# mikeferguson/ndt_2d

Hardware: AMD Instinct MI355X
Metric: pose-candidates x beams scored per second (higher is better)
Workload: dtype f64

## Files before the change

### experiments/asm_loop_mix.py

```python
#!/usr/bin/env python3
import collections
import hashlib
import json
import os
import re
import subprocess
import sys
import tempfile

R = os.path.dirname(os.path.dirname(os.path.abspath(__file__)))
KERNELS = [
    ("ndt2d_match_lane.hip", "match_lane_compact_kernel", r"25match_lane_compact_kernelILb1ELb1EEE"),
    ("ndt2d_match_lane.hip", "match_lane_compact_parts_kernel", r"31match_lane_compact_parts_kernelILb1EEE"),
    ("ndt2d_match_small.hip", "match_small_kernel", r"18match_small_kernelILb1ELb1ELb1EEE"),
    ("ndt2d_poses_compact.hip", "score_poses_compact_kernel", r"26score_poses_compact_kernelILi256ELb1ELb1ELb0EEE"),
]


def kernel_lines(path, pattern):
    out, on = [], False
    for line in open(path):
        if not on:
            if re.match(r"^_Z\w*%s\w*:" % pattern, line):
                on = True
            continue
        out.append(line)
        if line.strip().startswith("s_endpgm"):
            break
# ... 139 lines not shown
```

### experiments/lane_path_mix.py

```python
#!/usr/bin/env python3
import json
import os
import sys

R = os.path.dirname(os.path.dirname(os.path.abspath(__file__)))
paths_file = sys.argv[1] if len(sys.argv) > 1 else os.path.join(R, "profiles", "r06_lane_paths.json")
pmc_file = sys.argv[2] if len(sys.argv) > 2 else os.path.join(R, "profiles", "r06_pmc.json")
issue = json.load(open(os.path.join(R, "profiles", "r05_ubench_issue.json")))
CYC = issue["cycles"]
CLS = {k: ([c for c in v.get("counted_by", []) if not c.startswith("(")] or ["other"])[0]
       for k, v in issue["instructions"].items()}

P = {
    "lookup_group (per 8 beams)": [("v_add_f64", 8), ("v_perm_b32", 8), ("v_max_u32", 1), ("v_max3_u32", 3),
                                    ("v_cmp_le_u32 vcc", 1)],
    "live_group (8 live tests)": [("v_cmp_le_u32 vcc", 8)],
    "live_beam": [("v_and_b32", 1), ("v_cmp_le_u32 vcc", 1)],
    "near_test": [("v_cmp_gt_u16 vcc", 2), ("v_perm_b32", 1)],
    "exact_evaluation": [("v_add_f64", 2),
                         ("v_lshrrev_b32_sdwa", 2), ("v_mul_u32_u24", 1), ("v_add3_u32", 1), ("v_cndmask_b32 sgpr", 1),
                         ("v_lshl_add_u32", 1), ("v_mad_u32_u24", 1),
                         ("v_add_f64", 5), ("v_mul_f64", 6), ("v_cmp_lt_f64 vcc", 1)],
    "reference_index (extra)": [("v_add_f64", 2), ("v_mul_f64", 2), ("v_cmp_lt_f64 vcc", 4), ("v_cvt_u32_f64", 2),
                                ("v_mad_u64_u32", 1), ("v_mov_b32 from sgpr", 1), ("v_cndmask_b32 vcc", 1),
                                ("v_lshrrev_b32_sdwa", -2), ("v_mul_u32_u24", -1), ("v_add3_u32", -1),
                                ("v_cndmask_b32 sgpr", -1)],
    "exp_and_add": [("v_max_f64", 1), ("v_mul_f64", 1), ("v_rndne_f64", 1), ("v_fmac_f64", 2), ("v_fma_f64", 11),
                    ("v_cvt_i32_f64", 1), ("v_cmp_lt_f64 vcc", 1), ("v_ldexp_f64", 1), ("v_add_f64", 1)],
    "skip_refresh": [("v_frexp_exp_i32_f64", 1), ("v_add_u32", 2), ("v_mov_b32", 2), ("v_cvt_f64_i32", 1),
                     ("v_fma_f64", 1), ("v_cmp_lt_f64 vcc", 2), ("v_cndmask_b32 vcc", 2), ("v_ceil_f64", 1),
                     ("v_cvt_i32_f64", 1), ("v_max_u32", 1), ("v_min_u32", 1), ("v_lshlrev_b32", 1)],
}

doc = json.load(open(paths_file))
n = doc["counts"]
execs = {
    "lookup_group (per 8 beams)": n["beams_in_lookup_groups"] / 8.0,
    "live_group (8 live tests)": n["groups_with_a_live_lane"],
    "live_beam": n["beams_with_a_live_lane"],
    "near_test": n["live_beams_near_possible"],
    "exact_evaluation": n["exact_evaluations"],
# ... 57 lines not shown
```

### ndt_2d_amd/build.py

```python
import os
import subprocess
import sys

_PKG = os.path.dirname(os.path.abspath(__file__))
_ROOT = os.path.dirname(_PKG)
_CSRC = os.path.join(_PKG, "csrc")
LIB_PATH = os.path.join(_PKG, "libndt2d_hip.so")

BUILD_INFO_SOURCE = "ndt2d_build_info.cpp"
SOURCES = ["ndt2d_kernels.hip", "ndt2d_match_lane.hip", "ndt2d_match_small.hip", "ndt2d_poses_compact.hip", "ndt2d_build.hip", "ndt2d_motion.hip", "ndt2d_scan.hip", "ndt2d_occupancy.hip", "ndt2d_exchange.hip",
           "device/ndt2d_context.hip", "device/ndt2d_context_grid.hip", "device/ndt2d_context_search.hip", "device/ndt2d_context_poses.hip", "device/ndt2d_context_scan.hip",
           "resample/ndt2d_resample.hip", "occupancy_map/ndt2d_occupancy_map.hip", "seed/ndt2d_seed.hip", "clearance/ndt2d_clearance.hip", "cluster/ndt2d_cluster.hip", "build_small/ndt2d_build_small.hip", "closure/ndt2d_closure.hip", "starts/ndt2d_starts.hip", "wide/ndt2d_wide.hip", "scans/ndt2d_scans.hip", "refine/ndt2d_refine.hip", "verify/ndt2d_verify.hip", "posegraph/ndt2d_posegraph.hip", "posegraph/ndt2d_posegraph_robust.hip", "posegraph/ndt2d_posegraph_marginals.hip", "covariance/ndt2d_covariance.hip", "direct/ndt2d_direct.hip", "sparse/ndt2d_sparse.hip", "sparsecov/ndt2d_sparsecov.hip", "ndt2d_host.cpp",
           "host/ndt2d_host_ndt.cpp", "host/ndt2d_multi.cpp", "host/ndt2d_batched.cpp", "host/ndt2d_kld.cpp", "host/ndt2d_synth.cpp"]
HEADERS = [os.path.join(_CSRC, "ndt2d_kernels.h"), os.path.join(_CSRC, "ndt2d_device_fn.h"), os.path.join(_CSRC, "ndt2d_lane_fn.h"), os.path.join(_CSRC, "ndt2d_near_bits.h"), os.path.join(_CSRC, "ndt2d_pretest_level.h"), os.path.join(_CSRC, "ndt2d_poses_fn.h"), os.path.join(_CSRC, "ndt2d_exchange.h"), os.path.join(_CSRC, "ndt2d_eigen2.h"), os.path.join(_CSRC, "build_small", "ndt2d_build_fn.h"), os.path.join(_CSRC, "build_small", "ndt2d_build_small_fn.h"), os.path.join(_CSRC, "ndt2d_workers.h"), os.path.join(_CSRC, "ndt2d_guard.h"), os.path.join(_CSRC, "batch", "ndt2d_sum_chunks.h"), os.path.join(_CSRC, "batch", "ndt2d_walk_fn.h"), os.path.join(_CSRC, "batch", "ndt2d_job_groups.h"), os.path.join(_CSRC, "batch", "ndt2d_stage_layout.h"), os.path.join(_CSRC, "batch", "ndt2d_batch_search.h"), os.path.join(_CSRC, "batch", "ndt2d_installed_map.h"), os.path.join(_CSRC, "batch", "ndt2d_batch_state.h"), os.path.join(_CSRC, "batch", "ndt2d_batch_host.h"), os.path.join(_CSRC, "batch", "ndt2d_refine_jobs.h"), os.path.join(_CSRC, "refine", "ndt2d_refine_step.h"), os.path.join(_CSRC, "verify", "ndt2d_verify_ray.h"), os.path.join(_CSRC, "posegraph", "ndt2d_posegraph_fn.h"), os.path.join(_CSRC, "posegraph", "ndt2d_posegraph_chain.h"), os.path.join(_CSRC, "posegraph", "ndt2d_posegraph_loss.h"), os.path.join(_CSRC, "posegraph", "ndt2d_posegraph_relative.h"), os.path.join(_CSRC, "posegraph", "ndt2d_posegraph_kernel.h"), os.path.join(_CSRC, "posegraph", "ndt2d_posegraph_state.h"), os.path.join(_CSRC, "posegraph", "ndt2d_posegraph_args.h"), os.path.join(_CSRC, "covariance", "ndt2d_covariance_plan.h"), os.path.join(_CSRC, "covariance", "ndt2d_covariance_kernel.h"), os.path.join(_CSRC, "covariance", "ndt2d_covariance_launch.h"), os.path.join(_CSRC, "direct", "ndt2d_direct_step.h"), os.path.join(_CSRC, "direct", "ndt2d_direct_plan.h"), os.path.join(_CSRC, "direct", "ndt2d_direct_kernel.h"), os.path.join(_CSRC, "sparse", "ndt2d_sparse_plan.h"), os.path.join(_CSRC, "sparse", "ndt2d_sparse_schur.h"), os.path.join(_CSRC, "sparse", "ndt2d_sparse_kernel.h"), os.path.join(_CSRC, "sparsecov", "ndt2d_sparsecov_plan.h"), os.path.join(_CSRC, "sparsecov", "ndt2d_sparsecov_select.h"), os.path.join(_CSRC, "sparsecov", "ndt2d_sparsecov_kernel.h"), os.path.join(_CSRC, "seed", "ndt2d_seed_fn.h"), os.path.join(_CSRC, "clearance", "ndt2d_clearance_fn.h"), os.path.join(_CSRC, "cluster", "ndt2d_cluster_fn.h"), os.path.join(_CSRC, "wide", "ndt2d_wide_fn.h"), os.path.join(_CSRC, "closure", "ndt2d_closure_jobs.h"), os.path.join(_CSRC, "host", "ndt2d_host_ndt.h"), os.path.join(_CSRC, "host", "ndt2d_matcher_state.h"), os.path.join(_CSRC, "host", "ndt2d_job_batch.h"), os.path.join(_CSRC, "device", "ndt2d_context.h"), os.path.join(_CSRC, "refine", "ndt2d_refine_kernel.h"), os.path.join(_CSRC, "verify", "ndt2d_verify_kernel.h"), os.path.join(_CSRC, "particles", "ndt2d_philox.h"), os.path.join(_CSRC, "particles", "ndt2d_compact_fn.h"), os.path.join(_CSRC, "particles", "ndt2d_compact.h"), os.path.join(_CSRC, "particles", "ndt2d_key_table.h"), os.path.join(_CSRC, "particles", "ndt2d_device_object.h"), os.path.join(_ROOT, "include", "ndt2d_hip.h")]
ARCH = "gfx950"
FLAGS = ["-O3", "-std=c++17", "-ffp-contract=off", "-fPIC", "-Wall", "-Wextra",
         "-Wno-unused-parameter"]


SHA_MARKER = b"NDT2D_SOURCE_SHA256="


def source_sha256():
    import hashlib
    h = hashlib.sha256()
    paths = [os.path.join(_CSRC, s) for s in SOURCES + [BUILD_INFO_SOURCE]] + HEADERS
    for path in sorted(paths, key=os.path.basename):
        h.update(os.path.basename(path).encode() + b"\0")
        with open(path, "rb") as f:
# ... 178 lines not shown
```

### ndt_2d_amd/csrc/ndt2d_lane_fn.h

```cpp
#ifndef NDT2D_LANE_FN_H_
#define NDT2D_LANE_FN_H_

#include <cmath>

#include "ndt2d_device_fn.h"
#include "ndt2d_near_bits.h"
#include "ndt2d_pretest_level.h"

namespace ndt2d
{

namespace
{

constexpr int kPatch = 8;
#ifndef NDT2D_LANE_UNROLL
#define NDT2D_LANE_UNROLL 8
#endif
constexpr int kUnroll = NDT2D_LANE_UNROLL;
#ifndef NDT2D_LANE_NEAR_BITS
#define NDT2D_LANE_NEAR_BITS 1
#endif
constexpr double kFracScale = 65536.0;
constexpr int kMapStride = 256;
constexpr int kMaxMapCells = 256;
constexpr double kBoxMargin = 1.0 / 1024.0;
constexpr double kTwo24 = 16777216.0;
constexpr double kTwo52 = 4503599627370496.0;
constexpr double kNearBias = kNearUnits * (kTwo24 + 1.0);
static_assert(kNearUnits == 4 && kNearPatch == kPatch, "near_boundary() tests the biased fraction against 2 * kNearUnits");

struct LaneGeom
{
  int32_t pad;
// ... 272 lines not shown
  do {                                                                                        \
    if (g_lane_hist != nullptr && (threadIdx.x & 63u) == 0) atomicAdd(g_lane_hist + (slot), static_cast<double>(amount)); \
  } while (0)
#else
#define NDT2D_PATH(slot, amount) do {} while (0)
#endif

struct LaneCtx
{
  uint32_t rank_address;
  uint32_t lds_cells_address;
  uint32_t sub_log2;
  uint32_t exact_index;
  uint32_t idx_bias;
  uint32_t size_x;
};

__device__ __forceinline__ uint32_t lds_byte_at(uint32_t address)
{
  typedef const __attribute__((address_space(3))) uint8_t * lds_byte_ptr;
  return *reinterpret_cast<lds_byte_ptr>(address);
}

__device__ __forceinline__ uint32_t lds_u16_at(uint32_t address)
{
  typedef const __attribute__((address_space(3))) uint16_t * lds_u16_ptr;
  return *reinterpret_cast<lds_u16_ptr>(address);
}

__device__ __forceinline__ uint64_t near_boundary(uint32_t v)
{
  uint64_t lanes;
  asm("v_cmp_gt_u16_e64 %0, 8, %1" : "=s"(lanes) : "v"(v));
  return lanes;
}

__device__ __forceinline__ uint2 lds_two_dwords_at(uint32_t address)
{
  typedef const __attribute__((address_space(3), aligned(4))) uint32_t * lds_u32_ptr;
  const lds_u32_ptr p = reinterpret_cast<lds_u32_ptr>(address);
  return make_uint2(p[0], p[1]);
}
// ... 59 lines not shown
  v = min(v, __builtin_amdgcn_update_dpp(v, v, kDppRowMirror, 0xf, 0xf, false));
  v = min(v, __builtin_amdgcn_update_dpp(v, v, kDppRowBcast15, 0xa, 0xf, false));
  v = min(v, __builtin_amdgcn_update_dpp(v, v, kDppRowBcast31, 0xc, 0xf, false));
  return static_cast<uint32_t>(__builtin_amdgcn_readlane(v, kWave - 1));
}

__device__ __forceinline__ double lds_record_exponent(uint32_t cells_address, uint32_t idx,
                                                      double px, double py)
{
  typedef const __attribute__((address_space(3), aligned(16))) double * lds_double_ptr;
  const lds_double_ptr rec = reinterpret_cast<lds_double_ptr>(
    __umul24(idx, static_cast<uint32_t>(kCellDoubles * sizeof(double))) + cells_address);
  return record_exponent(rec[0], rec[1], rec[2], rec[3], rec[4], px, py);
}

struct SkipState
{
  double skip_below;
  uint32_t skip_level;
};

__device__ __forceinline__ SkipState skip_state(double sum, int32_t no_skip)
{
  SkipState s;
  if (no_skip)
  {
    s.skip_below = -HUGE_VAL;
    s.skip_level = 0;
    return s;
  }
  s.skip_below = negligible_below(sum);
  const int32_t l = static_cast<int32_t>(ceil(s.skip_below)) + 63;
  s.skip_level = static_cast<uint32_t>(min(max(l, 1), 63)) << 2;
  return s;
}

template <int U, bool POW2, bool LDS_RECORDS, bool SCALAR_ROWS = true, bool COMPACT = false>
__device__ __forceinline__ bool lane_beams(const GridDesc & g, const LaneCtx & c,
                                           const double4 (&o)[U], double dx, double dy,
                                           double dxy, double & sum, SkipState & skip,
                                           int32_t no_skip, uint32_t near_possible = ~0u)
{
  const double skip_below = skip.skip_below;
  const uint32_t skip_level = skip.skip_level;
  uint32_t lo[U], hi[U], m[U];
  uint32_t top = 0;
#pragma unroll
  for (int u = 0; u < U; ++u)
  {
    const double s = o[u].z + dxy;
    lo[u] = static_cast<uint32_t>(__double2loint(s));
    hi[u] = static_cast<uint32_t>(__double2hiint(s));
// ... 27 lines not shown
            (near_boundary(lo[u]) | near_boundary(fy) | ((no_skip | c.exact_index) != 0 ? ~0ull : 0ull)) & live_mask;
        }
        const uint64_t occ_lanes = __builtin_amdgcn_ballot_w64(occ);
        const uint64_t occ_mask = occ_lanes & live_mask;
#ifdef NDT2D_LANE_NO_EXACT
        if ((occ_mask | near_mask) == 0x1234567ull)
#else
        if ((occ_mask | near_mask) != 0ull)
#endif
        {
          NDT2D_PATH(205, 1);
          if (near_mask != 0ull) NDT2D_PATH(206, 1);
          const double px = o[u].x + dx;
          const double py = o[u].y + dy;
          uint32_t idx;
          if (near_mask != 0ull)
          {
            idx = cell_index<POW2>(g, px, py);
          }
          else
          {
            const uint32_t col = ((lo[u] >> 16) & 0xffu) >> c.sub_log2;
            const uint32_t row = ((hi[u] >> 8) & 0xffu) >> c.sub_log2;
            const uint32_t cell = __umul24(row, c.size_x) + (col - c.idx_bias);
            if (COMPACT)
            {
              asm("v_cndmask_b32 %0, -1, %1, %2" : "=v"(idx) : "v"(cell), "s"(occ_lanes));
            }
            else
            {
              idx = occ ? cell : g.ncell;
            }
          }
          if (COMPACT) idx = lds_u16_at(c.rank_address + 2u * idx);
          const double e = LDS_RECORDS ? lds_record_exponent(c.lds_cells_address, idx, px, py)
                                       : indexed_exponent<false>(g, nullptr, idx, px, py);
#ifdef NDT2D_LANE_HIST
          if (g_lane_hist != nullptr)
          {
            const uint64_t flagged = occ_mask | near_mask;
            const uint64_t needed = __builtin_amdgcn_ballot_w64(!(e < skip_below)) & flagged;
            if ((threadIdx.x & 63u) == 0)
            {
              atomicAdd(g_lane_hist + __popcll(flagged), 1.0);
              atomicAdd(g_lane_hist + 70 + __popcll(needed), 1.0);
              atomicAdd(g_lane_hist + (needed != 0ull ? 140 : 141), 1.0);
            }
          }
#endif
          if (wave_any(!(e < skip_below)))
          {
// ... 124 lines not shown
```

### ndt_2d_amd/csrc/ndt2d_match_lane.hip

```cpp
#include <cmath>
#include <cstdlib>

#include <type_traits>

#include "ndt2d_lane_fn.h"

namespace ndt2d
{

namespace
{

constexpr uint32_t kDynamicItemsFromBeams = 256;
constexpr int kLaneThreads = 1024;
constexpr int kLaneThreadsSmall = 256;
#ifndef NDT2D_LANE_THREADS_COMPACT
#define NDT2D_LANE_THREADS_COMPACT 768
#endif
constexpr int kLaneThreadsCompact = NDT2D_LANE_THREADS_COMPACT;
#define NDT2D_LANE_COMPACT_WAVES_PER_EU (NDT2D_LANE_THREADS_COMPACT / 128)

#ifndef NDT2D_LANE_TABLE_2D
#define NDT2D_LANE_TABLE_2D 1
#endif
// ... 124 lines not shown

__device__ __forceinline__ double packed_offset(double dx, double dy, double inv_scaled)
{
  return rint(dy * inv_scaled) * kTwo24 + rint(dx * inv_scaled);
}

__device__ __forceinline__ double no_index_here()
{
  static_assert(kNoIndex == 1.0e308, "the literal below is 1.0e308");
  uint32_t lo, hi;
  asm volatile("v_mov_b32 %0, 0x85ebc8a0\n\tv_mov_b32 %1, 0x7fe1ccf3" : "=v"(lo), "=v"(hi));
  return __hiloint2double(static_cast<int>(hi), static_cast<int>(lo));
}

template <int THREADS, bool POW2, bool LDS_RECORDS, bool DYNAMIC_ITEMS, bool COMPACT, bool PARTS = false,
          bool STRIPS = false, bool NEAR = false>
__device__ __forceinline__ void match_lane_body(
  const MatchArgs & a, const double4 * __restrict__ outer, const uint8_t * __restrict__ map_image,
  const LaneGeom & geo)
{
  extern __shared__ __align__(16) double lds[];
  const GridDesc & g = a.grid;
#if defined(NDT2D_LANE_HIST) || defined(NDT2D_LANE_PATHS)
  if (blockIdx.x == 0 && threadIdx.x == 0) g_lane_hist = a.scores;
#endif
  uint8_t * lds_map = reinterpret_cast<uint8_t *>(lds);
  const uint32_t map_bytes = static_cast<uint32_t>(geo.map_h) * kMapStride;
  const uint32_t rank_bytes = COMPACT ? compact_rank_bytes(g.ncell) : 0u;
  double * lds_cells = lds + (map_bytes + rank_bytes) / sizeof(double);

  if (COMPACT)
  {
    const uint4 * src_rank = reinterpret_cast<const uint4 *>(g.cell_rank);
    uint4 * dst_rank = reinterpret_cast<uint4 *>(lds_map + map_bytes + kRankLead);
    for (uint32_t i = threadIdx.x; i < (rank_bytes - kRankLead) / 16; i += THREADS) dst_rank[i] = src_rank[i];
    if (threadIdx.x == 0)
    {
      reinterpret_cast<uint16_t *>(lds_map + map_bytes + kRankLead)[-1] = static_cast<uint16_t>(g.n_occ);
    }
    const uint32_t n2 = (g.n_occ + 1) * kCellDoubles / 2;
    const double2 * src = reinterpret_cast<const double2 *>(g.compact_records);
    double2 * dst = reinterpret_cast<double2 *>(lds_cells);
    for (uint32_t i = threadIdx.x; i < n2; i += THREADS) dst[i] = src[i];
  }
  else if (LDS_RECORDS)
  {
    stage_grid_to_lds(g, lds_cells);
  }
  {
    const uint32_t n16 = static_cast<uint32_t>(kMapStride) * geo.map_h / 16;
    const uint4 * src = reinterpret_cast<const uint4 *>(map_image);
    uint4 * dst = reinterpret_cast<uint4 *>(lds_map);
    for (uint32_t i = threadIdx.x; i < n16; i += THREADS) dst[i] = src[i];
// ... 1 lines not shown
  __syncthreads();

#ifdef NDT2D_LANE_TRACE
  const unsigned long long trace_t0 = wall_clock64();
  unsigned long long trace_last = trace_t0, trace_max = 0, trace_last_start = trace_t0;
  uint32_t trace_items = 0, trace_prev_item = 0, trace_flagged = 0;
#endif
  LaneCtx c;
  c.rank_address = map_bytes + (COMPACT ? kRankLead : 0u);
  c.lds_cells_address = map_bytes + rank_bytes;
  c.sub_log2 = static_cast<uint32_t>(geo.sub_log2);
  c.exact_index = geo.block_log2 > 0 ? 1u : 0u;
  c.idx_bias = static_cast<uint32_t>(geo.pad - geo.win_y0) * g.size_x +
               static_cast<uint32_t>(geo.pad - geo.win_x0);
  c.size_x = g.size_x;

  const uint32_t lane = threadIdx.x & (kWave - 1);
  const uint32_t wave = __builtin_amdgcn_readfirstlane(threadIdx.x >> 6);
  const uint32_t n_lin = a.n_lin;
  static_assert(!STRIPS || (DYNAMIC_ITEMS && !PARTS), "strip tiles: the unsplit dynamic-item forms only");
  const LaneTiling tiling = lane_tiling(n_lin, STRIPS);
  const uint32_t patches = tiling.per_theta;
  const uint32_t n_items = (a.th_end - a.th_begin) * patches * (PARTS ? a.beam_parts : 1u);
  constexpr uint32_t kLaneWaves = THREADS / kWave;
  const uint32_t n_workers = gridDim.x * kLaneWaves;
  const uint32_t worker = wave * gridDim.x + blockIdx.x;
  const uint64_t per_theta = static_cast<uint64_t>(n_lin) * n_lin;
  const uint32_t th_mid = (a.th_end - a.th_begin - 1u) / 2u;
  const uint32_t home_shard = blockIdx.x % kItemShards;
  const double inv_scaled = geo.inv_scaled;
// ... 104 lines not shown
          }
        }
      }
#ifdef NDT2D_LANE_TRACE
      trace_flagged += static_cast<uint32_t>(__popcll(can_score));
#endif
      const uint32_t chunk_end = min(b0 + static_cast<uint32_t>(kWave), beams_end);
      uint32_t b = b0;
      for (; b + kUnroll <= chunk_end; b += kUnroll, can_score >>= kUnroll, near_chunk >>= kUnroll)
      {
        if ((can_score & ((1ull << kUnroll) - 1ull)) == 0ull) continue;
        double4 o[kUnroll];
#pragma unroll
        for (int u = 0; u < kUnroll; ++u) o[u] = row[b + u];
        __builtin_amdgcn_s_setprio(3);
        if (lane_beams<kUnroll, POW2, LDS_RECORDS, true, COMPACT>(g, c, o, dx, dy, dxy, sum, skip, geo.no_skip,
                                                                  NEAR ? static_cast<uint32_t>(near_chunk) : ~0u))
        {
          level_min |= 1u;
        }
        __builtin_amdgcn_s_setprio(0);
      }
      for (; b < chunk_end; ++b, can_score >>= 1, near_chunk >>= 1)
      {
        if ((can_score & 1ull) == 0ull) continue;
        const double4 one[1] = {row[b]};
        if (lane_beams<1, POW2, LDS_RECORDS, true, COMPACT>(g, c, one, dx, dy, dxy, sum, skip, geo.no_skip,
                                                            NEAR ? static_cast<uint32_t>(near_chunk) : ~0u))
        {
          level_min |= 1u;
        }
      }
    }

    if (PARTS)
    {
      a.part_sums[static_cast<size_t>(item) * kWave + lane] = sum;
      uint32_t next = n_items;
      if (lane == kWave - 1)
      {
        for (uint32_t tried = 0; tried < kItemShards && next >= n_items; ++tried)
        {
          const uint32_t shard = (home_shard + tried) % kItemShards;
// ... 132 lines not shown
      out[1] = best_i;
#pragma unroll
      for (int k = 0; k < 10; ++k) out[2 + k] = acc[k];
    }
  }
}

template <int THREADS, bool POW2, bool LDS_RECORDS, bool DYNAMIC_ITEMS, bool STRIPS = false>
__global__ void __launch_bounds__(THREADS) match_lane_kernel(
  const MatchArgs a, const double4 * __restrict__ outer, const uint8_t * __restrict__ map_image,
  const LaneGeom geo)
{
  match_lane_body<THREADS, POW2, LDS_RECORDS, DYNAMIC_ITEMS, false, false, STRIPS>(a, outer, map_image, geo);
}

template <bool STRIPS, bool NEAR>
__global__ void __launch_bounds__(kLaneThreadsCompact) __attribute__((amdgpu_waves_per_eu(NDT2D_LANE_COMPACT_WAVES_PER_EU)))
match_lane_compact_kernel(const MatchArgs a, const double4 * __restrict__ outer,
                          const uint8_t * __restrict__ map_image, const LaneGeom geo)
{
  match_lane_body<kLaneThreadsCompact, true, true, true, true, false, STRIPS, NEAR>(a, outer, map_image, geo);
}

template <bool POW2, bool STRIPS, bool NEAR>
__global__ void __launch_bounds__(kLaneThreadsCompact) __attribute__((amdgpu_waves_per_eu(NDT2D_LANE_COMPACT_WAVES_PER_EU)))
match_lane_gather6_kernel(const MatchArgs a, const double4 * __restrict__ outer,
                          const uint8_t * __restrict__ map_image, const LaneGeom geo)
{
  match_lane_body<kLaneThreadsCompact, POW2, false, true, false, false, STRIPS, NEAR>(a, outer, map_image, geo);
}

template <bool NEAR>
__global__ void __launch_bounds__(kLaneThreadsCompact) __attribute__((amdgpu_waves_per_eu(NDT2D_LANE_COMPACT_WAVES_PER_EU)))
match_lane_compact_parts_kernel(const MatchArgs a, const double4 * __restrict__ outer,
                                const uint8_t * __restrict__ map_image, const LaneGeom geo)
{
  match_lane_body<kLaneThreadsCompact, true, true, true, true, true, false, NEAR>(a, outer, map_image, geo);
}

template <bool POW2, bool NEAR>
__global__ void __launch_bounds__(kLaneThreadsCompact) __attribute__((amdgpu_waves_per_eu(NDT2D_LANE_COMPACT_WAVES_PER_EU)))
match_lane_gather6_parts_kernel(const MatchArgs a, const double4 * __restrict__ outer,
                                const uint8_t * __restrict__ map_image, const LaneGeom geo)
{
  match_lane_body<kLaneThreadsCompact, POW2, false, true, false, true, false, NEAR>(a, outer, map_image, geo);
}

__global__ void __launch_bounds__(256) match_lane_combine_kernel(const MatchArgs a)
{
  const uint32_t lane = threadIdx.x & (kWave - 1);
  const uint32_t n_lin = a.n_lin;
  const uint32_t patches_1d = (n_lin + kPatch - 1) / kPatch;
// ... 183 lines not shown
  args.part_beams = part_beams;
  if (!(dynamic_items && beam_parts == 1)) geo.strips = 0;
  const bool strips = geo.strips != 0;
  const uint64_t n_tiles =
    static_cast<uint64_t>(args.th_end - args.th_begin) * lane_tiling(args.n_lin, geo.strips != 0).per_theta;
  const uint64_t n_sub_items = beam_parts > 1 ? n_items * beam_parts : n_tiles;

  const bool small = beam_parts == 1 && n_items <= static_cast<uint64_t>(cus) * (kLaneThreadsSmall / kWave);
  const uint32_t waves_per_block = (small ? kLaneThreadsSmall : kLaneThreads) / kWave;
  uint32_t blocks = static_cast<uint32_t>((n_tiles + waves_per_block - 1) / waves_per_block);
  uint32_t max_blocks = static_cast<uint32_t>(cus);
  if (max_blocks * waves_per_block > max_workers) max_blocks = max_workers / waves_per_block;
  if (blocks > max_blocks) blocks = max_blocks;
  if (blocks == 0) blocks = 1;
  const bool compact = !small && compact_possible;
  const bool gather6 = !compact && !small && gather6_possible;
  if (records_mode_out != nullptr)
  {
    *records_mode_out = (compact ? 2 : (lds_records ? 1 : 0)) | (geo.block_log2 > 0 ? 4 : 0);
  }
  if (compact || gather6)
  {
    lds_bytes = compact ? map_bytes + compact_bytes : map_bytes;
    const uint32_t wpb = kLaneThreadsCompact / kWave;
    blocks = static_cast<uint32_t>((n_sub_items + wpb - 1) / wpb);
    uint32_t cap = 2 * static_cast<uint32_t>(cus);
    if (cap * wpb > max_workers) cap = max_workers / wpb;
    if (blocks > cap) blocks = cap;
    if (blocks == 0) blocks = 1;
  }
#if NDT2D_LANE_TABLE_2D
  {
    const uint32_t beam_blocks = (args.n_beams + 255u) / 256u;
    const uint32_t map_blocks = static_cast<uint32_t>(map_bytes + 255) / 256u;
    uint32_t th_rows = args.th_end - args.th_begin;
    if (beam_blocks == 0 || th_rows == 0) return hipErrorInvalidValue;
    const uint32_t map_rows = (map_blocks + beam_blocks - 1u) / beam_blocks;
    if (map_rows >= kTableMaxRows) return hipErrorInvalidValue;
// ... 24 lines not shown
  auto pick = [&](auto threads_tag) -> hipError_t {
    constexpr int T = decltype(threads_tag)::value;
    auto with_items = [&](auto dyn_tag, auto strips_tag) -> hipError_t {
      constexpr bool D = decltype(dyn_tag)::value;
      constexpr bool S = decltype(strips_tag)::value;
      return lds_records ? (pow2 ? launch(match_lane_kernel<T, true, true, D, S>, T)
                                 : launch(match_lane_kernel<T, false, true, D, S>, T))
                         : (pow2 ? launch(match_lane_kernel<T, true, false, D, S>, T)
                                 : launch(match_lane_kernel<T, false, false, D, S>, T));
    };
    if (!dynamic_items) return with_items(std::false_type{}, std::false_type{});
    return strips ? with_items(std::true_type{}, std::true_type{}) : with_items(std::true_type{}, std::false_type{});
  };
  auto six_wave = [&](auto near_tag) -> hipError_t {
    constexpr bool N = decltype(near_tag)::value;
    if (beam_parts > 1)
    {
      return compact ? launch(match_lane_compact_parts_kernel<N>, kLaneThreadsCompact)
                     : (pow2 ? launch(match_lane_gather6_parts_kernel<true, N>, kLaneThreadsCompact)
                             : launch(match_lane_gather6_parts_kernel<false, N>, kLaneThreadsCompact));
    }
    if (compact)
    {
      return strips ? launch(match_lane_compact_kernel<true, N>, kLaneThreadsCompact)
                    : launch(match_lane_compact_kernel<false, N>, kLaneThreadsCompact);
    }
    return pow2 ? (strips ? launch(match_lane_gather6_kernel<true, true, N>, kLaneThreadsCompact)
                          : launch(match_lane_gather6_kernel<true, false, N>, kLaneThreadsCompact))
                : (strips ? launch(match_lane_gather6_kernel<false, true, N>, kLaneThreadsCompact)
                          : launch(match_lane_gather6_kernel<false, false, N>, kLaneThreadsCompact));
  };
  const bool near = lane_reads_near_bits(geo, args.n_lin);
  if (beam_parts > 1)
  {
    e = near ? six_wave(std::true_type{}) : six_wave(std::false_type{});
    if (e == hipSuccess)
    {
      hipLaunchKernelGGL(match_lane_combine_kernel, dim3(static_cast<uint32_t>((n_items + 3) / 4)), dim3(256),
                         0, stream, args);
      e = hipGetLastError();
// ... 22 lines not shown
```

Measured before the change: 3253 billion.

## Address compacted LDS records through a precomputed window address table

Builds an LDS table over the padded search window whose entries hold either the direct LDS byte address of each cell's compacted record (4-byte entries) or its rank (1-byte entries when there are at most 256 records). The lane loop can then take a cell's record address from one LDS load instead of computing a linear cell index, looking up a 16-bit rank and scaling it. The aim is to cut integer address arithmetic and one dependent LDS lookup from the hot beam loop. In exchange the block uses more LDS, which can lower occupancy, and pays a table build at kernel start; the table is chosen only when it fits and can be turned off by an environment knob.

```diff
diff --git a/experiments/asm_loop_mix.py b/experiments/asm_loop_mix.py
--- a/experiments/asm_loop_mix.py
+++ b/experiments/asm_loop_mix.py
@@ -10,8 +10,8 @@
 
 R = os.path.dirname(os.path.dirname(os.path.abspath(__file__)))
 KERNELS = [
-    ("ndt2d_match_lane.hip", "match_lane_compact_kernel", r"25match_lane_compact_kernelILb1ELb1EEE"),
-    ("ndt2d_match_lane.hip", "match_lane_compact_parts_kernel", r"31match_lane_compact_parts_kernelILb1EEE"),
+    ("ndt2d_match_lane.hip", "match_lane_compact_kernel", r"25match_lane_compact_kernelILb1ELb1ELj1EEE"),
+    ("ndt2d_match_lane.hip", "match_lane_compact_parts_kernel", r"31match_lane_compact_parts_kernelILb1ELj1EEE"),
     ("ndt2d_match_small.hip", "match_small_kernel", r"18match_small_kernelILb1ELb1ELb1EEE"),
     ("ndt2d_poses_compact.hip", "score_poses_compact_kernel", r"26score_poses_compact_kernelILi256ELb1ELb1ELb0EEE"),
 ]
diff --git a/experiments/lane_path_mix.py b/experiments/lane_path_mix.py
--- a/experiments/lane_path_mix.py
+++ b/experiments/lane_path_mix.py
@@ -18,13 +18,12 @@
     "live_beam": [("v_and_b32", 1), ("v_cmp_le_u32 vcc", 1)],
     "near_test": [("v_cmp_gt_u16 vcc", 2), ("v_perm_b32", 1)],
     "exact_evaluation": [("v_add_f64", 2),
-                         ("v_lshrrev_b32_sdwa", 2), ("v_mul_u32_u24", 1), ("v_add3_u32", 1), ("v_cndmask_b32 sgpr", 1),
-                         ("v_lshl_add_u32", 1), ("v_mad_u32_u24", 1),
+                         ("v_lshrrev_b32_sdwa", 2), ("v_lshl_add_u32", 1), ("v_add_u32", 1), ("v_mad_u32_u24", 1),
                          ("v_add_f64", 5), ("v_mul_f64", 6), ("v_cmp_lt_f64 vcc", 1)],
     "reference_index (extra)": [("v_add_f64", 2), ("v_mul_f64", 2), ("v_cmp_lt_f64 vcc", 4), ("v_cvt_u32_f64", 2),
-                                ("v_mad_u64_u32", 1), ("v_mov_b32 from sgpr", 1), ("v_cndmask_b32 vcc", 1),
-                                ("v_lshrrev_b32_sdwa", -2), ("v_mul_u32_u24", -1), ("v_add3_u32", -1),
-                                ("v_cndmask_b32 sgpr", -1)],
+                                ("v_add_u32", 2), ("v_cmp_le_u32 vcc", 2), ("v_lshl_add_u32", 1),
+                                ("v_mov_b32 from sgpr", 1), ("v_cndmask_b32 vcc", 1),
+                                ("v_lshrrev_b32_sdwa", -2), ("v_lshl_add_u32", -1)],
     "exp_and_add": [("v_max_f64", 1), ("v_mul_f64", 1), ("v_rndne_f64", 1), ("v_fmac_f64", 2), ("v_fma_f64", 11),
                     ("v_cvt_i32_f64", 1), ("v_cmp_lt_f64 vcc", 1), ("v_ldexp_f64", 1), ("v_add_f64", 1)],
     "skip_refresh": [("v_frexp_exp_i32_f64", 1), ("v_add_u32", 2), ("v_mov_b32", 2), ("v_cvt_f64_i32", 1),
diff --git a/ndt_2d_amd/build.py b/ndt_2d_amd/build.py
--- a/ndt_2d_amd/build.py
+++ b/ndt_2d_amd/build.py
@@ -12,7 +12,7 @@
            "device/ndt2d_context.hip", "device/ndt2d_context_grid.hip", "device/ndt2d_context_search.hip", "device/ndt2d_context_poses.hip", "device/ndt2d_context_scan.hip",
            "resample/ndt2d_resample.hip", "occupancy_map/ndt2d_occupancy_map.hip", "seed/ndt2d_seed.hip", "clearance/ndt2d_clearance.hip", "cluster/ndt2d_cluster.hip", "build_small/ndt2d_build_small.hip", "closure/ndt2d_closure.hip", "starts/ndt2d_starts.hip", "wide/ndt2d_wide.hip", "scans/ndt2d_scans.hip", "refine/ndt2d_refine.hip", "verify/ndt2d_verify.hip", "posegraph/ndt2d_posegraph.hip", "posegraph/ndt2d_posegraph_robust.hip", "posegraph/ndt2d_posegraph_marginals.hip", "covariance/ndt2d_covariance.hip", "direct/ndt2d_direct.hip", "sparse/ndt2d_sparse.hip", "sparsecov/ndt2d_sparsecov.hip", "ndt2d_host.cpp",
            "host/ndt2d_host_ndt.cpp", "host/ndt2d_multi.cpp", "host/ndt2d_batched.cpp", "host/ndt2d_kld.cpp", "host/ndt2d_synth.cpp"]
-HEADERS = [os.path.join(_CSRC, "ndt2d_kernels.h"), os.path.join(_CSRC, "ndt2d_device_fn.h"), os.path.join(_CSRC, "ndt2d_lane_fn.h"), os.path.join(_CSRC, "ndt2d_near_bits.h"), os.path.join(_CSRC, "ndt2d_pretest_level.h"), os.path.join(_CSRC, "ndt2d_poses_fn.h"), os.path.join(_CSRC, "ndt2d_exchange.h"), os.path.join(_CSRC, "ndt2d_eigen2.h"), os.path.join(_CSRC, "build_small", "ndt2d_build_fn.h"), os.path.join(_CSRC, "build_small", "ndt2d_build_small_fn.h"), os.path.join(_CSRC, "ndt2d_workers.h"), os.path.join(_CSRC, "ndt2d_guard.h"), os.path.join(_CSRC, "batch", "ndt2d_sum_chunks.h"), os.path.join(_CSRC, "batch", "ndt2d_walk_fn.h"), os.path.join(_CSRC, "batch", "ndt2d_job_groups.h"), os.path.join(_CSRC, "batch", "ndt2d_stage_layout.h"), os.path.join(_CSRC, "batch", "ndt2d_batch_search.h"), os.path.join(_CSRC, "batch", "ndt2d_installed_map.h"), os.path.join(_CSRC, "batch", "ndt2d_batch_state.h"), os.path.join(_CSRC, "batch", "ndt2d_batch_host.h"), os.path.join(_CSRC, "batch", "ndt2d_refine_jobs.h"), os.path.join(_CSRC, "refine", "ndt2d_refine_step.h"), os.path.join(_CSRC, "verify", "ndt2d_verify_ray.h"), os.path.join(_CSRC, "posegraph", "ndt2d_posegraph_fn.h"), os.path.join(_CSRC, "posegraph", "ndt2d_posegraph_chain.h"), os.path.join(_CSRC, "posegraph", "ndt2d_posegraph_loss.h"), os.path.join(_CSRC, "posegraph", "ndt2d_posegraph_relative.h"), os.path.join(_CSRC, "posegraph", "ndt2d_posegraph_kernel.h"), os.path.join(_CSRC, "posegraph", "ndt2d_posegraph_state.h"), os.path.join(_CSRC, "posegraph", "ndt2d_posegraph_args.h"), os.path.join(_CSRC, "covariance", "ndt2d_covariance_plan.h"), os.path.join(_CSRC, "covariance", "ndt2d_covariance_kernel.h"), os.path.join(_CSRC, "covariance", "ndt2d_covariance_launch.h"), os.path.join(_CSRC, "direct", "ndt2d_direct_step.h"), os.path.join(_CSRC, "direct", "ndt2d_direct_plan.h"), os.path.join(_CSRC, "direct", "ndt2d_direct_kernel.h"), os.path.join(_CSRC, "sparse", "ndt2d_sparse_plan.h"), os.path.join(_CSRC, "sparse", "ndt2d_sparse_schur.h"), os.path.join(_CSRC, "sparse", "ndt2d_sparse_kernel.h"), os.path.join(_CSRC, "sparsecov", "ndt2d_sparsecov_plan.h"), os.path.join(_CSRC, "sparsecov", "ndt2d_sparsecov_select.h"), os.path.join(_CSRC, "sparsecov", "ndt2d_sparsecov_kernel.h"), os.path.join(_CSRC, "seed", "ndt2d_seed_fn.h"), os.path.join(_CSRC, "clearance", "ndt2d_clearance_fn.h"), os.path.join(_CSRC, "cluster", "ndt2d_cluster_fn.h"), os.path.join(_CSRC, "wide", "ndt2d_wide_fn.h"), os.path.join(_CSRC, "closure", "ndt2d_closure_jobs.h"), os.path.join(_CSRC, "host", "ndt2d_host_ndt.h"), os.path.join(_CSRC, "host", "ndt2d_matcher_state.h"), os.path.join(_CSRC, "host", "ndt2d_job_batch.h"), os.path.join(_CSRC, "device", "ndt2d_context.h"), os.path.join(_CSRC, "refine", "ndt2d_refine_kernel.h"), os.path.join(_CSRC, "verify", "ndt2d_verify_kernel.h"), os.path.join(_CSRC, "particles", "ndt2d_philox.h"), os.path.join(_CSRC, "particles", "ndt2d_compact_fn.h"), os.path.join(_CSRC, "particles", "ndt2d_compact.h"), os.path.join(_CSRC, "particles", "ndt2d_key_table.h"), os.path.join(_CSRC, "particles", "ndt2d_device_object.h"), os.path.join(_ROOT, "include", "ndt2d_hip.h")]
+HEADERS = [os.path.join(_CSRC, "ndt2d_kernels.h"), os.path.join(_CSRC, "ndt2d_device_fn.h"), os.path.join(_CSRC, "ndt2d_lane_fn.h"), os.path.join(_CSRC, "ndt2d_near_bits.h"), os.path.join(_CSRC, "ndt2d_address_table.h"), os.path.join(_CSRC, "ndt2d_pretest_level.h"), os.path.join(_CSRC, "ndt2d_poses_fn.h"), os.path.join(_CSRC, "ndt2d_exchange.h"), os.path.join(_CSRC, "ndt2d_eigen2.h"), os.path.join(_CSRC, "build_small", "ndt2d_build_fn.h"), os.path.join(_CSRC, "build_small", "ndt2d_build_small_fn.h"), os.path.join(_CSRC, "ndt2d_workers.h"), os.path.join(_CSRC, "ndt2d_guard.h"), os.path.join(_CSRC, "batch", "ndt2d_sum_chunks.h"), os.path.join(_CSRC, "batch", "ndt2d_walk_fn.h"), os.path.join(_CSRC, "batch", "ndt2d_job_groups.h"), os.path.join(_CSRC, "batch", "ndt2d_stage_layout.h"), os.path.join(_CSRC, "batch", "ndt2d_batch_search.h"), os.path.join(_CSRC, "batch", "ndt2d_installed_map.h"), os.path.join(_CSRC, "batch", "ndt2d_batch_state.h"), os.path.join(_CSRC, "batch", "ndt2d_batch_host.h"), os.path.join(_CSRC, "batch", "ndt2d_refine_jobs.h"), os.path.join(_CSRC, "refine", "ndt2d_refine_step.h"), os.path.join(_CSRC, "verify", "ndt2d_verify_ray.h"), os.path.join(_CSRC, "posegraph", "ndt2d_posegraph_fn.h"), os.path.join(_CSRC, "posegraph", "ndt2d_posegraph_chain.h"), os.path.join(_CSRC, "posegraph", "ndt2d_posegraph_loss.h"), os.path.join(_CSRC, "posegraph", "ndt2d_posegraph_relative.h"), os.path.join(_CSRC, "posegraph", "ndt2d_posegraph_kernel.h"), os.path.join(_CSRC, "posegraph", "ndt2d_posegraph_state.h"), os.path.join(_CSRC, "posegraph", "ndt2d_posegraph_args.h"), os.path.join(_CSRC, "covariance", "ndt2d_covariance_plan.h"), os.path.join(_CSRC, "covariance", "ndt2d_covariance_kernel.h"), os.path.join(_CSRC, "covariance", "ndt2d_covariance_launch.h"), os.path.join(_CSRC, "direct", "ndt2d_direct_step.h"), os.path.join(_CSRC, "direct", "ndt2d_direct_plan.h"), os.path.join(_CSRC, "direct", "ndt2d_direct_kernel.h"), os.path.join(_CSRC, "sparse", "ndt2d_sparse_plan.h"), os.path.join(_CSRC, "sparse", "ndt2d_sparse_schur.h"), os.path.join(_CSRC, "sparse", "ndt2d_sparse_kernel.h"), os.path.join(_CSRC, "sparsecov", "ndt2d_sparsecov_plan.h"), os.path.join(_CSRC, "sparsecov", "ndt2d_sparsecov_select.h"), os.path.join(_CSRC, "sparsecov", "ndt2d_sparsecov_kernel.h"), os.path.join(_CSRC, "seed", "ndt2d_seed_fn.h"), os.path.join(_CSRC, "clearance", "ndt2d_clearance_fn.h"), os.path.join(_CSRC, "cluster", "ndt2d_cluster_fn.h"), os.path.join(_CSRC, "wide", "ndt2d_wide_fn.h"), os.path.join(_CSRC, "closure", "ndt2d_closure_jobs.h"), os.path.join(_CSRC, "host", "ndt2d_host_ndt.h"), os.path.join(_CSRC, "host", "ndt2d_matcher_state.h"), os.path.join(_CSRC, "host", "ndt2d_job_batch.h"), os.path.join(_CSRC, "device", "ndt2d_context.h"), os.path.join(_CSRC, "refine", "ndt2d_refine_kernel.h"), os.path.join(_CSRC, "verify", "ndt2d_verify_kernel.h"), os.path.join(_CSRC, "particles", "ndt2d_philox.h"), os.path.join(_CSRC, "particles", "ndt2d_compact_fn.h"), os.path.join(_CSRC, "particles", "ndt2d_compact.h"), os.path.join(_CSRC, "particles", "ndt2d_key_table.h"), os.path.join(_CSRC, "particles", "ndt2d_device_object.h"), os.path.join(_ROOT, "include", "ndt2d_hip.h")]
 ARCH = "gfx950"
 FLAGS = ["-O3", "-std=c++17", "-ffp-contract=off", "-fPIC", "-Wall", "-Wextra",
          "-Wno-unused-parameter"]
diff --git a/ndt_2d_amd/csrc/ndt2d_address_table.h b/ndt_2d_amd/csrc/ndt2d_address_table.h
--- /dev/null
+++ b/ndt_2d_amd/csrc/ndt2d_address_table.h
@@ -0,0 +1,77 @@
+#ifndef NDT2D_ADDRESS_TABLE_H_
+#define NDT2D_ADDRESS_TABLE_H_
+
+#include <cstdint>
+
+#if defined(__HIPCC__) || defined(__CUDACC__)
+#define NDT2D_ADDRESS_HD __host__ __device__
+#else
+#define NDT2D_ADDRESS_HD
+#endif
+
+namespace ndt2d
+{
+
+struct AddressTableShape
+{
+  uint32_t rows;
+  uint32_t cols;
+  uint32_t stride_log2;
+};
+
+NDT2D_ADDRESS_HD inline AddressTableShape address_table_shape(int32_t win_w, int32_t win_h, int32_t pad)
+{
+  AddressTableShape s;
+  s.rows = static_cast<uint32_t>(win_h + 2 * pad);
+  s.cols = static_cast<uint32_t>(win_w + 2 * pad);
+  s.stride_log2 = 0;
+  while ((1u << s.stride_log2) < s.cols) ++s.stride_log2;
+  return s;
+}
+
+NDT2D_ADDRESS_HD inline uint32_t address_table_outside(const AddressTableShape & s) { return s.rows << s.stride_log2; }
+
+NDT2D_ADDRESS_HD inline uint32_t address_table_entries(const AddressTableShape & s) { return address_table_outside(s) + 1u; }
+
+constexpr uint32_t kAddressEntryBytes = 4;
+constexpr uint32_t kRankEntryBytes = 1;
+constexpr uint32_t kRankEntryMaxRecords = 256;
+
+NDT2D_ADDRESS_HD inline uint32_t address_table_bytes(const AddressTableShape & s, uint32_t entry_bytes)
+{
+  return (address_table_entries(s) * entry_bytes + 15u) & ~15u;
+}
+
+NDT2D_ADDRESS_HD inline uint32_t address_table_entry(const AddressTableShape & s, uint32_t col, uint32_t row)
+{
+  return (row << s.stride_log2) + col;
+}
+
+NDT2D_ADDRESS_HD inline uint32_t address_table_rank(const uint16_t * cell_rank, uint32_t size_x, uint32_t size_y,
+                                                    uint32_t n_occ, int32_t win_x0, int32_t win_y0, int32_t pad,
+                                                    const AddressTableShape & s, uint32_t entry)
+{
+  const uint32_t row = entry >> s.stride_log2;
+  const uint32_t col = entry & ((1u << s.stride_log2) - 1u);
+  if (row >= s.rows || col >= s.cols) return n_occ;
+  const int32_t cx = static_cast<int32_t>(col) - pad + win_x0;
+  const int32_t cy = static_cast<int32_t>(row) - pad + win_y0;
+  if (cx < 0 || cy < 0 || cx >= static_cast<int32_t>(size_x) || cy >= static_cast<int32_t>(size_y)) return n_occ;
+  return cell_rank[static_cast<uint32_t>(cy) * size_x + static_cast<uint32_t>(cx)];
+}
+
+NDT2D_ADDRESS_HD inline uint32_t address_table_value(uint32_t records_address, uint32_t rank, uint32_t record_bytes)
+{
+  return records_address + rank * record_bytes;
+}
+
+NDT2D_ADDRESS_HD inline uint32_t address_table_entry_of_cell(const AddressTableShape & s, uint32_t off_x,
+                                                             uint32_t off_y, bool inside, uint32_t gx, uint32_t gy)
+{
+  const uint32_t col = gx + off_x, row = gy + off_y;
+  return (inside && col < s.cols && row < s.rows) ? address_table_entry(s, col, row) : address_table_outside(s);
+}
+
+}
+
+#endif
diff --git a/ndt_2d_amd/csrc/ndt2d_lane_fn.h b/ndt_2d_amd/csrc/ndt2d_lane_fn.h
--- a/ndt_2d_amd/csrc/ndt2d_lane_fn.h
+++ b/ndt_2d_amd/csrc/ndt2d_lane_fn.h
@@ -3,6 +3,7 @@
 
 #include <cmath>
 
+#include "ndt2d_address_table.h"
 #include "ndt2d_device_fn.h"
 #include "ndt2d_near_bits.h"
 #include "ndt2d_pretest_level.h"
@@ -18,6 +19,9 @@
 #define NDT2D_LANE_UNROLL 8
 #endif
 constexpr int kUnroll = NDT2D_LANE_UNROLL;
+#ifndef NDT2D_LANE_ADDRESS_TABLE
+#define NDT2D_LANE_ADDRESS_TABLE 1
+#endif
 #ifndef NDT2D_LANE_NEAR_BITS
 #define NDT2D_LANE_NEAR_BITS 1
 #endif
@@ -320,6 +324,9 @@
   uint32_t exact_index;
   uint32_t idx_bias;
   uint32_t size_x;
+  uint32_t table_address;
+  AddressTableShape table;
+  uint32_t win_off_x, win_off_y;
 };
 
 __device__ __forceinline__ uint32_t lds_byte_at(uint32_t address)
@@ -332,6 +339,12 @@
 {
   typedef const __attribute__((address_space(3))) uint16_t * lds_u16_ptr;
   return *reinterpret_cast<lds_u16_ptr>(address);
+}
+
+__device__ __forceinline__ uint32_t lds_u32_at(uint32_t address)
+{
+  typedef const __attribute__((address_space(3), aligned(4))) uint32_t * lds_u32_ptr;
+  return *reinterpret_cast<lds_u32_ptr>(address);
 }
 
 __device__ __forceinline__ uint64_t near_boundary(uint32_t v)
@@ -421,6 +434,35 @@
   return record_exponent(rec[0], rec[1], rec[2], rec[3], rec[4], px, py);
 }
 
+__device__ __forceinline__ double lds_record_exponent_at(uint32_t record_address, double px, double py)
+{
+  typedef const __attribute__((address_space(3), aligned(16))) double * lds_double_ptr;
+  const lds_double_ptr rec = reinterpret_cast<lds_double_ptr>(record_address);
+  return record_exponent(rec[0], rec[1], rec[2], rec[3], rec[4], px, py);
+}
+
+template <bool POW2>
+__device__ __forceinline__ uint32_t window_table_entry(const GridDesc & g, const LaneCtx & c, double px, double py)
+{
+  const double tx = px - g.origin_x;
+  const double ty = py - g.origin_y;
+  double fx, fy;
+  if (POW2)
+  {
+    fx = tx * g.inv_cell_size;
+    fy = ty * g.inv_cell_size;
+  }
+  else
+  {
+    fx = tx / g.cell_size;
+    fy = ty / g.cell_size;
+  }
+  const bool inside = (tx >= 0.0) & (ty >= 0.0) & (fx < static_cast<double>(g.size_x)) &
+                      (fy < static_cast<double>(g.size_y));
+  return address_table_entry_of_cell(c.table, c.win_off_x, c.win_off_y, inside, static_cast<uint32_t>(fx),
+                                     static_cast<uint32_t>(fy));
+}
+
 struct SkipState
 {
   double skip_below;
@@ -442,7 +484,7 @@
   return s;
 }
 
-template <int U, bool POW2, bool LDS_RECORDS, bool SCALAR_ROWS = true, bool COMPACT = false>
+template <int U, bool POW2, bool LDS_RECORDS, bool SCALAR_ROWS = true, bool COMPACT = false, uint32_t TABLE = 0>
 __device__ __forceinline__ bool lane_beams(const GridDesc & g, const LaneCtx & c,
                                            const double4 (&o)[U], double dx, double dy,
                                            double dxy, double & sum, SkipState & skip,
@@ -500,7 +542,15 @@
           const double px = o[u].x + dx;
           const double py = o[u].y + dy;
           uint32_t idx;
-          if (near_mask != 0ull)
+          if (TABLE != 0)
+          {
+            static_assert(TABLE == 0 || (COMPACT && LDS_RECORDS), "the window table addresses the compacted LDS records");
+            static_assert(TABLE == 0 || TABLE == kAddressEntryBytes || TABLE == kRankEntryBytes, "entries of four bytes or one");
+            idx = near_mask != 0ull
+                    ? window_table_entry<POW2>(g, c, px, py)
+                    : address_table_entry(c.table, ((lo[u] >> 16) & 0xffu) >> c.sub_log2, ((hi[u] >> 8) & 0xffu) >> c.sub_log2);
+          }
+          else if (near_mask != 0ull)
           {
             idx = cell_index<POW2>(g, px, py);
           }
@@ -518,9 +568,12 @@
               idx = occ ? cell : g.ncell;
             }
           }
-          if (COMPACT) idx = lds_u16_at(c.rank_address + 2u * idx);
-          const double e = LDS_RECORDS ? lds_record_exponent(c.lds_cells_address, idx, px, py)
-                                       : indexed_exponent<false>(g, nullptr, idx, px, py);
+          if (COMPACT && TABLE == 0) idx = lds_u16_at(c.rank_address + 2u * idx);
+          if (TABLE == kRankEntryBytes) idx = lds_byte_at(c.table_address + idx);
+          const double e = TABLE == kAddressEntryBytes
+                             ? lds_record_exponent_at(lds_u32_at(c.table_address + 4u * idx), px, py)
+                             : LDS_RECORDS ? lds_record_exponent(c.lds_cells_address, idx, px, py)
+                                           : indexed_exponent<false>(g, nullptr, idx, px, py);
 #ifdef NDT2D_LANE_HIST
           if (g_lane_hist != nullptr)
           {
diff --git a/ndt_2d_amd/csrc/ndt2d_match_lane.hip b/ndt_2d_amd/csrc/ndt2d_match_lane.hip
--- a/ndt_2d_amd/csrc/ndt2d_match_lane.hip
+++ b/ndt_2d_amd/csrc/ndt2d_match_lane.hip
@@ -162,7 +162,7 @@
 }
 
 template <int THREADS, bool POW2, bool LDS_RECORDS, bool DYNAMIC_ITEMS, bool COMPACT, bool PARTS = false,
-          bool STRIPS = false, bool NEAR = false>
+          bool STRIPS = false, bool NEAR = false, uint32_t TABLE = 0>
 __device__ __forceinline__ void match_lane_body(
   const MatchArgs & a, const double4 * __restrict__ outer, const uint8_t * __restrict__ map_image,
   const LaneGeom & geo)
@@ -174,17 +174,40 @@
 #endif
   uint8_t * lds_map = reinterpret_cast<uint8_t *>(lds);
   const uint32_t map_bytes = static_cast<uint32_t>(geo.map_h) * kMapStride;
-  const uint32_t rank_bytes = COMPACT ? compact_rank_bytes(g.ncell) : 0u;
+  static_assert(TABLE == 0 || COMPACT, "the window table of record addresses: the compacted-records forms only");
+  const AddressTableShape table = address_table_shape(geo.win_w, geo.win_h, geo.pad);
+  const uint32_t rank_bytes = TABLE != 0 ? address_table_bytes(table, TABLE) : (COMPACT ? compact_rank_bytes(g.ncell) : 0u);
   double * lds_cells = lds + (map_bytes + rank_bytes) / sizeof(double);
 
   if (COMPACT)
   {
-    const uint4 * src_rank = reinterpret_cast<const uint4 *>(g.cell_rank);
-    uint4 * dst_rank = reinterpret_cast<uint4 *>(lds_map + map_bytes + kRankLead);
-    for (uint32_t i = threadIdx.x; i < (rank_bytes - kRankLead) / 16; i += THREADS) dst_rank[i] = src_rank[i];
-    if (threadIdx.x == 0)
-    {
-      reinterpret_cast<uint16_t *>(lds_map + map_bytes + kRankLead)[-1] = static_cast<uint16_t>(g.n_occ);
+    if (TABLE != 0)
+    {
+      const uint32_t n_entries = address_table_entries(table);
+      for (uint32_t i = threadIdx.x; i < n_entries; i += THREADS)
+      {
+        const uint32_t rank =
+          address_table_rank(g.cell_rank, g.size_x, g.size_y, g.n_occ, geo.win_x0, geo.win_y0, geo.pad, table, i);
+        if (TABLE == kRankEntryBytes)
+        {
+          lds_map[map_bytes + i] = static_cast<uint8_t>(rank);
+        }
+        else
+        {
+          reinterpret_cast<uint32_t *>(lds_map + map_bytes)[i] =
+            address_table_value(map_bytes + rank_bytes, rank, static_cast<uint32_t>(kCellDoubles * sizeof(double)));
+        }
+      }
+    }
+    else
+    {
+      const uint4 * src_rank = reinterpret_cast<const uint4 *>(g.cell_rank);
+      uint4 * dst_rank = reinterpret_cast<uint4 *>(lds_map + map_bytes + kRankLead);
+      for (uint32_t i = threadIdx.x; i < (rank_bytes - kRankLead) / 16; i += THREADS) dst_rank[i] = src_rank[i];
+      if (threadIdx.x == 0)
+      {
+        reinterpret_cast<uint16_t *>(lds_map + map_bytes + kRankLead)[-1] = static_cast<uint16_t>(g.n_occ);
+      }
     }
     const uint32_t n2 = (g.n_occ + 1) * kCellDoubles / 2;
     const double2 * src = reinterpret_cast<const double2 *>(g.compact_records);
@@ -216,6 +239,10 @@
   c.idx_bias = static_cast<uint32_t>(geo.pad - geo.win_y0) * g.size_x +
                static_cast<uint32_t>(geo.pad - geo.win_x0);
   c.size_x = g.size_x;
+  c.table_address = map_bytes;
+  c.table = table;
+  c.win_off_x = static_cast<uint32_t>(geo.pad - geo.win_x0);
+  c.win_off_y = static_cast<uint32_t>(geo.pad - geo.win_y0);
 
   const uint32_t lane = threadIdx.x & (kWave - 1);
   const uint32_t wave = __builtin_amdgcn_readfirstlane(threadIdx.x >> 6);
@@ -350,8 +377,8 @@
 #pragma unroll
         for (int u = 0; u < kUnroll; ++u) o[u] = row[b + u];
         __builtin_amdgcn_s_setprio(3);
-        if (lane_beams<kUnroll, POW2, LDS_RECORDS, true, COMPACT>(g, c, o, dx, dy, dxy, sum, skip, geo.no_skip,
-                                                                  NEAR ? static_cast<uint32_t>(near_chunk) : ~0u))
+        if (lane_beams<kUnroll, POW2, LDS_RECORDS, true, COMPACT, TABLE>(
+              g, c, o, dx, dy, dxy, sum, skip, geo.no_skip, NEAR ? static_cast<uint32_t>(near_chunk) : ~0u))
         {
           level_min |= 1u;
         }
@@ -361,8 +388,8 @@
       {
         if ((can_score & 1ull) == 0ull) continue;
         const double4 one[1] = {row[b]};
-        if (lane_beams<1, POW2, LDS_RECORDS, true, COMPACT>(g, c, one, dx, dy, dxy, sum, skip, geo.no_skip,
-                                                            NEAR ? static_cast<uint32_t>(near_chunk) : ~0u))
+        if (lane_beams<1, POW2, LDS_RECORDS, true, COMPACT, TABLE>(
+              g, c, one, dx, dy, dxy, sum, skip, geo.no_skip, NEAR ? static_cast<uint32_t>(near_chunk) : ~0u))
         {
           level_min |= 1u;
         }
@@ -525,12 +552,12 @@
   match_lane_body<THREADS, POW2, LDS_RECORDS, DYNAMIC_ITEMS, false, false, STRIPS>(a, outer, map_image, geo);
 }
 
-template <bool STRIPS, bool NEAR>
+template <bool STRIPS, bool NEAR, uint32_t TABLE>
 __global__ void __launch_bounds__(kLaneThreadsCompact) __attribute__((amdgpu_waves_per_eu(NDT2D_LANE_COMPACT_WAVES_PER_EU)))
 match_lane_compact_kernel(const MatchArgs a, const double4 * __restrict__ outer,
                           const uint8_t * __restrict__ map_image, const LaneGeom geo)
 {
-  match_lane_body<kLaneThreadsCompact, true, true, true, true, false, STRIPS, NEAR>(a, outer, map_image, geo);
+  match_lane_body<kLaneThreadsCompact, true, true, true, true, false, STRIPS, NEAR, TABLE>(a, outer, map_image, geo);
 }
 
 template <bool POW2, bool STRIPS, bool NEAR>
@@ -541,12 +568,12 @@
   match_lane_body<kLaneThreadsCompact, POW2, false, true, false, false, STRIPS, NEAR>(a, outer, map_image, geo);
 }
 
-template <bool NEAR>
+template <bool NEAR, uint32_t TABLE>
 __global__ void __launch_bounds__(kLaneThreadsCompact) __attribute__((amdgpu_waves_per_eu(NDT2D_LANE_COMPACT_WAVES_PER_EU)))
 match_lane_compact_parts_kernel(const MatchArgs a, const double4 * __restrict__ outer,
                                 const uint8_t * __restrict__ map_image, const LaneGeom geo)
 {
-  match_lane_body<kLaneThreadsCompact, true, true, true, true, true, false, NEAR>(a, outer, map_image, geo);
+  match_lane_body<kLaneThreadsCompact, true, true, true, true, true, false, NEAR, TABLE>(a, outer, map_image, geo);
 }
 
 template <bool POW2, bool NEAR>
@@ -760,6 +787,26 @@
   if (blocks > max_blocks) blocks = max_blocks;
   if (blocks == 0) blocks = 1;
   const bool compact = !small && compact_possible;
+  const AddressTableShape table_shape = address_table_shape(geo.win_w, geo.win_h, geo.pad);
+  const size_t records_bytes = (static_cast<size_t>(args.grid.n_occ) + 1) * kCellDoubles * sizeof(double);
+  const char * knob_table = std::getenv("NDT2D_LANE_ADDRESS_TABLE");
+  uint32_t table_entry_bytes = 0;
+  if (NDT2D_LANE_ADDRESS_TABLE != 0 && compact && geo.block_log2 == 0 && !(knob_table != nullptr && knob_table[0] == '0'))
+  {
+    if (2 * (map_bytes + address_table_bytes(table_shape, kAddressEntryBytes) + records_bytes) <= lds_per_block &&
+        !(knob_table != nullptr && knob_table[0] == '1'))
+    {
+      table_entry_bytes = kAddressEntryBytes;
+    }
+    else if (args.grid.n_occ + 1u <= kRankEntryMaxRecords &&
+             2 * (map_bytes + address_table_bytes(table_shape, kRankEntryBytes) + records_bytes) <= lds_per_block)
+    {
+      table_entry_bytes = kRankEntryBytes;
+    }
+  }
+  const bool address_table = table_entry_bytes != 0;
+  const size_t table_image_bytes =
+    map_bytes + (address_table ? address_table_bytes(table_shape, table_entry_bytes) : 0) + records_bytes;
   const bool gather6 = !compact && !small && gather6_possible;
   if (records_mode_out != nullptr)
   {
@@ -767,7 +814,7 @@
   }
   if (compact || gather6)
   {
-    lds_bytes = compact ? map_bytes + compact_bytes : map_bytes;
+    lds_bytes = compact ? (address_table ? table_image_bytes : map_bytes + compact_bytes) : map_bytes;
     const uint32_t wpb = kLaneThreadsCompact / kWave;
     blocks = static_cast<uint32_t>((n_sub_items + wpb - 1) / wpb);
     uint32_t cap = 2 * static_cast<uint32_t>(cus);
@@ -822,16 +869,30 @@
   };
   auto six_wave = [&](auto near_tag) -> hipError_t {
     constexpr bool N = decltype(near_tag)::value;
+    constexpr uint32_t A4 = NDT2D_LANE_ADDRESS_TABLE != 0 ? kAddressEntryBytes : 0u;
+    constexpr uint32_t A1 = NDT2D_LANE_ADDRESS_TABLE != 0 ? kRankEntryBytes : 0u;
+    if (compact && address_table && table_entry_bytes == kAddressEntryBytes)
+    {
+      if (beam_parts > 1) return launch(match_lane_compact_parts_kernel<N, A4>, kLaneThreadsCompact);
+      return strips ? launch(match_lane_compact_kernel<true, N, A4>, kLaneThreadsCompact)
+                    : launch(match_lane_compact_kernel<false, N, A4>, kLaneThreadsCompact);
+    }
+    if (compact && address_table)
+    {
+      if (beam_parts > 1) return launch(match_lane_compact_parts_kernel<N, A1>, kLaneThreadsCompact);
+      return strips ? launch(match_lane_compact_kernel<true, N, A1>, kLaneThreadsCompact)
+                    : launch(match_lane_compact_kernel<false, N, A1>, kLaneThreadsCompact);
+    }
     if (beam_parts > 1)
     {
-      return compact ? launch(match_lane_compact_parts_kernel<N>, kLaneThreadsCompact)
+      return compact ? launch(match_lane_compact_parts_kernel<N, 0u>, kLaneThreadsCompact)
                      : (pow2 ? launch(match_lane_gather6_parts_kernel<true, N>, kLaneThreadsCompact)
                              : launch(match_lane_gather6_parts_kernel<false, N>, kLaneThreadsCompact));
     }
     if (compact)
     {
-      return strips ? launch(match_lane_compact_kernel<true, N>, kLaneThreadsCompact)
-                    : launch(match_lane_compact_kernel<false, N>, kLaneThreadsCompact);
+      return strips ? launch(match_lane_compact_kernel<true, N, 0u>, kLaneThreadsCompact)
+                    : launch(match_lane_compact_kernel<false, N, 0u>, kLaneThreadsCompact);
     }
     return pow2 ? (strips ? launch(match_lane_gather6_kernel<true, true, N>, kLaneThreadsCompact)
                           : launch(match_lane_gather6_kernel<true, false, N>, kLaneThreadsCompact))
```

Result: faster. 3300 billion, median of 6 (+1.4%).
